# jonassibbesen/rpvg

Measured on AMD Instinct MI355X. Metric: read-pairs quantified/sec, higher is better.
Workload: dtype f64

## Files before the change

### rpvg_amd/csrc/subset_em.hip

```cpp

#include "common.hpp"

#include <cmath>
#include <memory>

using namespace rpvg_hip_detail;

namespace {

constexpr uint32_t kMaxSelected = 1024;

struct MergedList {
    const uint32_t * a;
    const uint32_t * b;
    uint32_t na, nb, i, j;
    __device__ __forceinline__ MergedList(const uint32_t * a_in, uint32_t na_in, const uint32_t * b_in, uint32_t nb_in)
        : a(a_in), b(b_in), na(na_in), nb(nb_in), i(0), j(0) {}
    __device__ __forceinline__ bool done() const { return i >= na && j >= nb; }
    __device__ __forceinline__ uint32_t next() {
        if (j >= nb || (i < na && a[i] <= b[j])) return a[i++];
        return b[j++];
    }
};

// ... 232 lines not shown
        for (uint32_t stride = size >> 1; stride > 0; stride >>= 1) {
            for (uint32_t i = threadIdx.x; i < padded; i += BLOCK) {
                const uint32_t partner = i ^ stride;
                if (partner > i) {
                    const bool ascending = (i & size) == 0;
                    const uint32_t x = order[i], y = order[partner];
                    if (before(y, x) == ascending) {
                        order[i] = y;
                        order[partner] = x;
                    }
                }
            }
            __syncthreads();
        }
    }
    const uint64_t slot0 = args.slot_off[m];
    unsigned long long my_subsets = 0, my_length = 0, my_columns = 0;
    for (uint32_t rank = threadIdx.x; rank < n_ret; rank += BLOCK) {
        const uint32_t s = order[rank];
        uint32_t distinct = 0, previous = 0xffffffffu;
        MergedList walk = columns.list(first[sel[s]], second[sel[s]]);
        while (!walk.done()) {
            const uint32_t path = walk.next();
            distinct += (path != previous) ? 1u : 0u;
            previous = path;
        }
        args.slot_first[slot0 + rank] = first[sel[s]];
        args.slot_second[slot0 + rank] = second[sel[s]];
        args.slot_weight[slot0 + rank] = weight[s];
        args.slot_length[slot0 + rank] = length[s];
        args.slot_columns[slot0 + rank] = distinct;
        my_subsets += 1;
        my_length += length[s];
        my_columns += distinct;
    }
    if (my_subsets) {
        atomicAdd(&red[0], my_subsets);
        atomicAdd(&red[1], my_length);
        atomicAdd(&red[2], my_columns);
    }
    __syncthreads();
    if (threadIdx.x == 0) {
        const uint64_t r0 = args.cluster_row_off[k], r1 = args.cluster_row_off[k + 1];
        const unsigned long long rows = r1 - r0, entries = args.row_ent_off[r1] - args.row_ent_off[r0];
        *out_totals = MatrixTotals{red[0], red[1], red[2], red[0] * rows, red[0] * entries, red[0] * ((rows + args.segment_rows - 1) / args.segment_rows)};
    }
}

__global__ __launch_bounds__(64) void subsetSelectSmallKernel(const SelectArgs args) {
    const uint32_t m = blockIdx.x;
    if (m >= args.num_matrices) return;
    if (args.pair_count[m] > kSmallSelected) {
        if (threadIdx.x == 0) args.big_matrices[atomicAdd(&args.header->big_count, 1u)] = m;
        return;
    }
    selectSubsetsOfMatrix<kSmallSelected, kSmallCachedPaths, 64>(args, m);
}

__global__ __launch_bounds__(256) void subsetSelectWideKernel(const SelectArgs args) {
    const uint32_t count = args.header->big_count;
    for (uint32_t item = blockIdx.x; item < count; item += gridDim.x) {
        selectSubsetsOfMatrix<kMaxSelected, kWideCachedPaths, 256>(args, args.big_matrices[item]);
        __syncthreads();
    }
}

struct OffsetsArgs {
    const uint32_t * pair_count;
    const unsigned long long * log_evals;
    const uint32_t * build_error;
    uint32_t num_matrices;
    const MatrixTotals * totals;
    MatrixTotals * bases;
    SubsetHeader * header;
    unsigned long long cap_subsets, cap_length, cap_columns, cap_rows, cap_entries, cap_items;
    uint64_t * seg_first;
    uint64_t * path_off;
    uint64_t * col_off;
};

__global__ __launch_bounds__(1024) void subsetOffsetsKernel(const OffsetsArgs args) {
    __shared__ MatrixTotals sums[1024];
    const uint32_t M = args.num_matrices;
    const uint32_t per = (M + 1023) / 1024;
    const uint32_t lo = min(M, threadIdx.x * per), hi = min(M, lo + per);
    MatrixTotals mine{0, 0, 0, 0, 0, 0};
    unsigned long long my_pairs = 0;
    for (uint32_t m = lo; m < hi; ++m) {
        my_pairs += args.pair_count[m];
        const MatrixTotals t = args.totals[m];
        mine.subsets += t.subsets;
        mine.list_length += t.list_length;
        mine.columns += t.columns;
        mine.rows += t.rows;
        mine.entries += t.entries;
        mine.segments += t.segments;
    }
    sums[threadIdx.x] = mine;
    if (my_pairs) atomicAdd(&args.header->kept_pairs, my_pairs);
    __syncthreads();
    for (uint32_t step = 1; step < 1024; step <<= 1) {
        MatrixTotals add{0, 0, 0, 0, 0, 0};
        if (threadIdx.x >= step) add = sums[threadIdx.x - step];
        __syncthreads();
        MatrixTotals & s = sums[threadIdx.x];
        s.subsets += add.subsets;
        s.list_length += add.list_length;
        s.columns += add.columns;
        s.rows += add.rows;
        s.entries += add.entries;
        s.segments += add.segments;
        __syncthreads();
    }
    MatrixTotals run = sums[threadIdx.x];
    run.subsets -= mine.subsets;
    run.list_length -= mine.list_length;
    run.columns -= mine.columns;
    run.rows -= mine.rows;
    run.entries -= mine.entries;
    run.segments -= mine.segments;
    for (uint32_t m = lo; m < hi; ++m) {
        args.bases[m] = run;
        const MatrixTotals t = args.totals[m];
        run.subsets += t.subsets;
        run.list_length += t.list_length;
        run.columns += t.columns;
        run.rows += t.rows;
        run.entries += t.entries;
        run.segments += t.segments;
    }
    if (threadIdx.x == 1023) {
        const MatrixTotals all = sums[1023];
        SubsetHeader * h = args.header;
        h->subsets = all.subsets;
        h->list_length = all.list_length;
        h->columns = all.columns;
        h->rows = all.rows;
        h->entries = all.entries;
        h->segments = all.segments;
        const bool fits = h->select_overflow == 0 && all.subsets <= args.cap_subsets && all.list_length <= args.cap_length &&
                          all.columns <= args.cap_columns && all.rows <= args.cap_rows && all.entries <= args.cap_entries &&
                          all.segments <= args.cap_items && all.subsets < 0xffffffffull && all.segments < 0xffffffffull;
        h->overflow = fits ? 0ull : 1ull;
        h->num_problems = fits ? static_cast<uint32_t>(all.subsets) : 0u;
        h->num_items = fits ? static_cast<uint32_t>(all.segments) : 0u;
        h->log_evals = *args.log_evals;
        h->build_bad = args.build_error ? *args.build_error : 0u;
        if (fits) {
            args.path_off[all.subsets] = all.list_length;
            args.col_off[all.subsets] = all.columns;
            args.seg_first[all.subsets] = all.segments;
        }
    }
}

struct ExpandArgs {
    uint32_t num_matrices;
    const SubsetHeader * header;
    const MatrixTotals * totals;
    const MatrixTotals * bases;
    const uint64_t * slot_off;
    const uint32_t * slot_first;
    const uint32_t * slot_second;
    const double * slot_weight;
    const uint32_t * slot_length;
    const uint32_t * slot_columns;
    const uint64_t * group_off;
    const uint64_t * group_path_off;
    const uint32_t * group_path;
    const uint32_t * cluster;
    const uint64_t * cluster_row_off;
    const uint64_t * row_ent_off;
    uint32_t * sub_cluster;
    double * sub_weight;
    uint64_t * path_off;
    uint32_t * path;
    uint64_t * col_off;
    uint32_t * col_path;
    uint64_t * row_base;
    uint64_t * ent_base;
    uint64_t * seg_first;
    uint32_t * item_problem;
    uint32_t segment_rows;
    uint64_t * subset_off;
};

__global__ __launch_bounds__(256) void subsetExpandKernel(const ExpandArgs args) {
    constexpr int BLOCK = 256;
    __shared__ uint32_t scratch[BLOCK / 64];
    const uint32_t m = blockIdx.x;
    if (m >= args.num_matrices) return;
    const MatrixTotals base = args.bases[m];
    if (threadIdx.x == 0) {
        args.subset_off[m] = args.header->overflow ? 0 : base.subsets;
        if (m + 1 == args.num_matrices) args.subset_off[m + 1] = args.header->overflow ? 0 : args.header->subsets;
    }
    if (args.header->overflow) return;
    const uint32_t n = static_cast<uint32_t>(args.totals[m].subsets);
    const uint64_t slot0 = args.slot_off[m];
    const Columns columns{args.group_path_off, args.group_path, args.group_off[m]};
    const uint32_t k = args.cluster[m];
    const uint64_t r0 = args.cluster_row_off[k], r1 = args.cluster_row_off[k + 1];
    const uint64_t rows = r1 - r0, entries = args.row_ent_off[r1] - args.row_ent_off[r0];
    uint64_t length_run = base.list_length, columns_run = base.columns;
    for (uint32_t c = 0; c < n; c += BLOCK) {
        const uint32_t r = c + threadIdx.x;
        const uint32_t len = r < n ? args.slot_length[slot0 + r] : 0u, cols = r < n ? args.slot_columns[slot0 + r] : 0u;
        uint32_t len_total, cols_total;
        const uint32_t len_before = blockExclusiveScan<BLOCK>(len, len_total, scratch);
        const uint32_t cols_before = blockExclusiveScan<BLOCK>(cols, cols_total, scratch);
        if (r < n) {
            const uint64_t s = base.subsets + r;
            const uint64_t p0 = length_run + len_before, c0 = columns_run + cols_before;
            args.sub_cluster[s] = k;
            args.sub_weight[s] = args.slot_weight[slot0 + r];
            args.path_off[s] = p0;
            args.col_off[s] = c0;
            args.row_base[s] = base.rows + static_cast<uint64_t>(r) * rows;
            args.ent_base[s] = base.entries + static_cast<uint64_t>(r) * entries;
            const uint64_t segments = (rows + args.segment_rows - 1) / args.segment_rows, item0 = base.segments + static_cast<uint64_t>(r) * segments;
            args.seg_first[s] = item0;
            for (uint64_t item = item0; item < item0 + segments; ++item) args.item_problem[item] = static_cast<uint32_t>(s);
            MergedList list = columns.list(args.slot_first[slot0 + r], args.slot_second[slot0 + r]);
            uint32_t previous = 0xffffffffu;
            uint64_t pw = p0, cw = c0;
            while (!list.done()) {
                const uint32_t path = list.next();
                args.path[pw++] = path;
                if (path != previous) args.col_path[cw++] = path;
                previous = path;
            }
        }
        length_run += len_total;
        columns_run += cols_total;
    }
}

struct PackArgs {
    const SubsetHeader * header;
    uint32_t num_matrices;
    const uint64_t * subset_off;
    const double * weight;
    const uint64_t * path_off;
    const uint64_t * col_off;
    const double * abundances;
    const double * noise;
    const double * total;
    const uint32_t * path;
    const uint32_t * col_path;
    const uint32_t * iterations;
    const uint32_t * kept_rows;
    const uint32_t * kept_entries;
    const uint32_t * merge_bad;
    unsigned char * packed;
};

__global__ __launch_bounds__(256) void packResultsKernel(const PackArgs args) {
    const SubsetHeader h = *args.header;
    if (h.overflow) return;
    const uint64_t M = args.num_matrices, S = h.subsets, L = h.list_length, C = h.columns;
    const PackedLayout lay = packedLayout(M, S, L, C);
    const size_t stride = static_cast<size_t>(gridDim.x) * blockDim.x, first = static_cast<size_t>(blockIdx.x) * blockDim.x + threadIdx.x;
    auto copy = [&](const size_t offset, const void * from, const size_t words) {
        uint32_t * to = reinterpret_cast<uint32_t *>(args.packed + offset);
        const uint32_t * src = static_cast<const uint32_t *>(from);
        for (size_t i = first; i < words; i += stride) to[i] = src[i];
    };
    copy(lay.subset_off, args.subset_off, (M + 1) * 2);
    copy(lay.weight, args.weight, S * 2);
    copy(lay.path_off, args.path_off, (S + 1) * 2);
    copy(lay.col_off, args.col_off, (S + 1) * 2);
    copy(lay.abundances, args.abundances, C * 2);
    copy(lay.noise, args.noise, S * 2);
    copy(lay.total, args.total, S * 2);
    copy(lay.path, args.path, L);
    copy(lay.col_path, args.col_path, C);
    copy(lay.iterations, args.iterations, S);
    copy(lay.kept_rows, args.kept_rows, S);
    copy(lay.kept_entries, args.kept_entries, S);
    if (args.merge_bad && first == 0) *reinterpret_cast<uint32_t *>(args.packed + lay.merge_flags) = *args.merge_bad;
}

constexpr uint32_t kMergeLdsRecords = 2048;
constexpr unsigned long long kMergeNoRecord = ~0ull;
constexpr uint32_t kMergePathBits = 27, kMergeRankBits = 10;

struct MergeArgs {
    const SubsetHeader * header;
    uint32_t num_matrices;
    const uint64_t * subset_off;
    const double * weight;
    const uint64_t * path_off;
    const uint32_t * path;
    const uint64_t * col_off;
    const uint32_t * col_path;
    const double * abundances;
    const double * noise;
    const double * total;
    const uint32_t * cluster;
    const uint64_t * cluster_path_off;
    const uint32_t * path_group_id;
    unsigned long long * sort_key;
    uint32_t * sort_pos;
    double * rec_a0;
    double * rec_a1;
    uint32_t * merge_bad;
// ... 180 lines not shown
    uint32_t max_paths = 0;
    std::vector<uint64_t> slot_off(M + 1, 0);
    for (uint32_t m = 0; m < M; ++m) {
        const uint64_t G = groups->h_num_cols[m];
        slot_off[m + 1] = slot_off[m] + std::min<uint64_t>(G * (G + 1) / 2, kMaxSelected);
        const uint32_t k = groups->h_cluster[m];
        lane_rows += batch->h_cluster_row_off[k + 1] - batch->h_cluster_row_off[k];
        lane_entries += batch->h_cluster_ent_off[k + 1] - batch->h_cluster_ent_off[k];
        lane_paths += groups->h_num_paths[m];
        max_paths = std::max(max_paths, groups->h_num_paths[m]);
        max_cluster_work = std::max<uint64_t>(max_cluster_work, (batch->h_cluster_row_off[k + 1] - batch->h_cluster_row_off[k]) +
                                                                    (batch->h_cluster_ent_off[k + 1] - batch->h_cluster_ent_off[k]));
    }
    slots = slot_off[M];
    if (M > 0 && 8ull * (5ull * (static_cast<uint64_t>(max_paths) + 1) + 6) > 156 * 1024) {
        setError("rpvg_hip_nested_subset_em: not taken (a cluster with %u paths: EM vectors in global memory)", max_paths);
        return RPVG_HIP_ERR_UNSUPPORTED;
    }

    std::lock_guard<std::mutex> lock(ctx->mutex);
    RPVG_HIP_CHECK(hipSetDevice(ctx->device));
    hipStream_t st = ctx->stream;
    if (M == 0) {
        *result_out = res.release();
        return RPVG_HIP_OK;
    }
    SubsetEmHints & hints = ctx->subset_hints;
    auto planned = [](const double per_unit, const unsigned long long units, const double headroom) {
        return static_cast<unsigned long long>(std::ceil(per_unit * headroom * static_cast<double>(units)));
    };
    unsigned long long cap_subsets = std::min<unsigned long long>(slots, hints.subsets_per_matrix > 0 ? planned(hints.subsets_per_matrix, M, 1.25) + 256 : std::max<unsigned long long>(8ull * M, 16384));
    unsigned long long cap_length = std::max<unsigned long long>(planned(hints.list_per_path, lane_paths, 2.0), std::max<unsigned long long>(8 * lane_paths, 1u << 20));
    unsigned long long cap_rows = hints.rows_per_row > 0 ? planned(hints.rows_per_row, lane_rows, 1.25) + 65536 : 8 * lane_rows;
    unsigned long long cap_entries = hints.entries_per_entry > 0 ? planned(hints.entries_per_entry, lane_entries, 1.25) + 65536 : 8 * lane_entries;
    if (hints.retry) {
        cap_subsets = std::min<unsigned long long>(slots, std::max(cap_subsets, hints.retry_subsets + 64));
        cap_length = std::max(cap_length, hints.retry_list_length + 64);
        cap_rows = std::max(cap_rows, hints.retry_rows + 64);
        cap_entries = std::max(cap_entries, hints.retry_entries + 64);
        hints.retry = false;
    }
    const unsigned long long cap_columns = cap_length;
    const unsigned long long cap_items = cap_rows / emFillSegmentRows() + cap_subsets;

    scope.reset(new HostScope("subset em: search + kernels queued"));
    const size_t header_room = 256;
    int rc = RPVG_HIP_OK;
    if (!second_attempt) {
        search.extra_u64 = slot_off.data();
        search.extra_u64_count = M + 1;
        search.extra_zero_bytes = header_room + emQueuesBytes();
        rc = queuePairSearch(ctx, groups, column_counts, min_rel_likelihood, search);
        if (rc != RPVG_HIP_OK) return rc;
    } else {
        const hipError_t zeroed = zeroAsync(search.d_extra_zero.ptr, search.extra_zero_bytes, st);
        if (zeroed != hipSuccess) {
            setError("rpvg_hip_nested_subset_em: %s", hipGetErrorString(zeroed));
            return RPVG_HIP_ERR_RUNTIME;
        }
    }

    hipError_t e = hipSuccess;
    auto ok = [&](hipError_t r) { if (e == hipSuccess) e = r; return e == hipSuccess; };
    const uint64_t * d_slot_off = search.d_extra_u64.ptr;
    SubsetHeader * header = reinterpret_cast<SubsetHeader *>(search.d_extra_zero.ptr);
    static_assert(sizeof(SubsetHeader) <= 256, "room for the header");
    DeviceBuffer<uint32_t> d_slot_first, d_slot_second, d_slot_length, d_slot_columns;
    DeviceBuffer<double> d_slot_weight;
    DeviceBuffer<unsigned char> d_totals, d_bases, d_packed;
    ok(d_slot_first.alloc(slots));
    ok(d_slot_second.alloc(slots));
    ok(d_slot_length.alloc(slots));
    ok(d_slot_columns.alloc(slots));
    ok(d_slot_weight.alloc(slots));
    ok(d_totals.alloc(sizeof(MatrixTotals) * M));
    ok(d_bases.alloc(sizeof(MatrixTotals) * M));
    DeviceBuffer<uint32_t> d_big_matrices;
    ok(d_big_matrices.alloc(M));
    DeviceBuffer<uint32_t> d_sub_cluster, d_path, d_col_path, d_iters, d_kept_rows, d_kept_entries;
    DeviceBuffer<double> d_sub_weight, d_abund, d_noise, d_total;
    DeviceBuffer<uint64_t> d_path_off, d_col_off, d_row_base, d_ent_base, d_subset_off, d_seg_first;
    DeviceBuffer<uint32_t> d_item_problem;
    ok(d_sub_cluster.alloc(cap_subsets));
    ok(d_sub_weight.alloc(cap_subsets));
    ok(d_path_off.alloc(cap_subsets + 1));
    ok(d_col_off.alloc(cap_subsets + 1));
    ok(d_row_base.alloc(cap_subsets));
    ok(d_ent_base.alloc(cap_subsets));
    ok(d_subset_off.alloc(M + 1));
    ok(d_seg_first.alloc(cap_subsets + 1));
    ok(d_item_problem.alloc(cap_items));
    ok(d_path.alloc(cap_length));
    ok(d_col_path.alloc(cap_columns));
    ok(d_abund.alloc(cap_columns));
    ok(d_noise.alloc(cap_subsets));
    ok(d_total.alloc(cap_subsets));
    ok(d_iters.alloc(cap_subsets));
    ok(d_kept_rows.alloc(cap_subsets));
    ok(d_kept_entries.alloc(cap_subsets));
    const size_t packed_capacity = packedLayout(M, cap_subsets, cap_length, cap_columns).bytes;
    ok(d_packed.alloc(packed_capacity));
    const bool merge_here = batch->path_group_id.ptr != nullptr && max_paths < (1u << kMergePathBits) - 2;
    DeviceBuffer<unsigned long long> d_merge_key;
    DeviceBuffer<uint32_t> d_merge_pos;
    DeviceBuffer<double> d_merge_a0, d_merge_a1;
    if (merge_here) {
        ok(d_merge_key.alloc(2 * cap_length + 2));
        ok(d_merge_pos.alloc(2 * cap_length + 2));
        ok(d_merge_a0.alloc(cap_length));
        ok(d_merge_a1.alloc(cap_length));
    }
    void * pinned_header = nullptr;
    if (e == hipSuccess && pinnedAlloc(&pinned_header, sizeof(SubsetHeader)) != hipSuccess) e = hipErrorOutOfMemory;
    hipEvent_t header_here = nullptr;
    if (e == hipSuccess) ok(hipEventCreateWithFlags(&header_here, hipEventDisableTiming));
    if (e != hipSuccess) {
        setError("rpvg_hip_nested_subset_em: %s", hipGetErrorString(e));
        (void) hipStreamSynchronize(st);
        leavePairSearch(ctx);
        if (pinned_header) pinnedFree(pinned_header);
        if (header_here) (void) hipEventDestroy(header_here);
        return (e == hipErrorOutOfMemory) ? RPVG_HIP_ERR_ALLOC : RPVG_HIP_ERR_RUNTIME;
    }
    MatrixTotals * totals = reinterpret_cast<MatrixTotals *>(d_totals.ptr);
    MatrixTotals * bases = reinterpret_cast<MatrixTotals *>(d_bases.ptr);

    std::unique_ptr<HostScope> part_scope(new HostScope("subset em: select + offsets + expand queued"));
    int span = ctx->spanBegin(FAM_BUILD);
    SelectArgs sa;
    sa.num_matrices = M;
    sa.pair_count = search.d_tail.ptr;
    sa.pair_cap_off = search.d_pair_cap_off.ptr;
    sa.pair_first = search.d_out_first.ptr;
    sa.pair_second = search.d_out_second.ptr;
    sa.pair_value = search.d_out_value.ptr;
    sa.group_off = groups->d_group_off;
    sa.group_path_off = groups->d_group_path_off;
    sa.group_path = groups->d_group_path;
    sa.cluster = groups->d_cluster;
    sa.mat_rows = groups->mat_rows.ptr;
    sa.cluster_row_off = batch->cluster_row_off.ptr;
    sa.row_ent_off = batch->row_ent_off.ptr;
    sa.slot_off = d_slot_off;
    sa.min_hap_prob = min_hap_prob;
    sa.segment_rows = emFillSegmentRows();
    sa.slot_first = d_slot_first.ptr;
    sa.slot_second = d_slot_second.ptr;
    sa.slot_weight = d_slot_weight.ptr;
    sa.slot_length = d_slot_length.ptr;
    sa.slot_columns = d_slot_columns.ptr;
    sa.totals = totals;
    sa.header = header;
    sa.big_matrices = d_big_matrices.ptr;
    subsetSelectSmallKernel<<<dim3(M), dim3(64), 0, st>>>(sa);
    subsetSelectWideKernel<<<dim3(std::min<uint32_t>(M, 128)), dim3(256), 0, st>>>(sa);
    const bool check_build = !groups->build_checked && groups->build_error_flag.ptr;
    OffsetsArgs oa;
    oa.pair_count = search.d_tail.ptr;
    oa.log_evals = reinterpret_cast<const unsigned long long *>(search.d_tail.ptr + search.evals_word);
    oa.build_error = check_build ? groups->build_error_flag.ptr : nullptr;
    oa.num_matrices = M;
    oa.totals = totals;
    oa.bases = bases;
    oa.header = header;
    oa.cap_subsets = cap_subsets;
    oa.cap_length = cap_length;
    oa.cap_columns = cap_columns;
    oa.cap_rows = cap_rows;
    oa.cap_entries = cap_entries;
    oa.cap_items = cap_items;
    oa.seg_first = d_seg_first.ptr;
    oa.path_off = d_path_off.ptr;
    oa.col_off = d_col_off.ptr;
    subsetOffsetsKernel<<<dim3(1), dim3(1024), 0, st>>>(oa);
    SubsetHeader * h_header = static_cast<SubsetHeader *>(pinned_header);
    ok(hipMemcpyAsync(h_header, header, sizeof(SubsetHeader), hipMemcpyDeviceToHost, st));
    ok(hipEventRecord(header_here, st));
    ExpandArgs ea;
    ea.num_matrices = M;
    ea.header = header;
    ea.totals = totals;
    ea.bases = bases;
    ea.slot_off = d_slot_off;
    ea.slot_first = d_slot_first.ptr;
    ea.slot_second = d_slot_second.ptr;
    ea.slot_weight = d_slot_weight.ptr;
    ea.slot_length = d_slot_length.ptr;
    ea.slot_columns = d_slot_columns.ptr;
    ea.group_off = groups->d_group_off;
    ea.group_path_off = groups->d_group_path_off;
    ea.group_path = groups->d_group_path;
    ea.cluster = groups->d_cluster;
    ea.cluster_row_off = batch->cluster_row_off.ptr;
    ea.row_ent_off = batch->row_ent_off.ptr;
    ea.sub_cluster = d_sub_cluster.ptr;
    ea.sub_weight = d_sub_weight.ptr;
    ea.path_off = d_path_off.ptr;
    ea.path = d_path.ptr;
    ea.col_off = d_col_off.ptr;
    ea.col_path = d_col_path.ptr;
    ea.row_base = d_row_base.ptr;
    ea.ent_base = d_ent_base.ptr;
    ea.seg_first = d_seg_first.ptr;
    ea.item_problem = d_item_problem.ptr;
    ea.segment_rows = emFillSegmentRows();
    ea.subset_off = d_subset_off.ptr;
    subsetExpandKernel<<<dim3(M), dim3(256), 0, st>>>(ea);
    ok(hipGetLastError());
    ctx->spanEnd(span);
    ctx->stats.build_launches += 4;
    leavePairSearch(ctx);

    part_scope.reset();
    EmProblemList list;
    list.P_bound = static_cast<uint32_t>(std::min<unsigned long long>(cap_subsets, 0xfffffffeull));
    list.d_num_problems = &header->num_problems;
    list.d_cluster = d_sub_cluster.ptr;
    list.d_col_off = d_col_off.ptr;
    list.d_col_path = d_col_path.ptr;
    list.d_row_base = d_row_base.ptr;
    list.d_ent_base = d_ent_base.ptr;
    list.rows_capacity = cap_rows;
    list.entries_capacity = cap_entries;
    list.d_seg_first = d_seg_first.ptr;
    list.d_item_problem = d_item_problem.ptr;
    list.items_bound = static_cast<uint32_t>(std::min<unsigned long long>(cap_items, 0xfffffffeull));
    list.d_num_items = &header->num_items;
    list.max_cols = max_paths + 1;
    list.max_cluster_paths = max_paths;
    list.max_cluster_work = max_cluster_work;
    list.wide_capacity = 0;
    EmOutputs out{d_abund.ptr, d_noise.ptr, d_iters.ptr, d_kept_rows.ptr, d_kept_entries.ptr, d_total.ptr};
    EmSolveWork work;
    work.zeroed_queues = search.d_extra_zero.ptr + header_room;
    if (e == hipSuccess) {
        rc = queueEmSolve(ctx, batch, list, max_em_its, max_rel_em_conv, out, work, false, collapse_precision);
        if (rc != RPVG_HIP_OK) {
            (void) hipStreamSynchronize(st);
            (void) hipEventDestroy(header_here);
            pinnedFree(pinned_header);
            return rc;
        }
    }
    part_scope.reset(new HostScope("subset em: merge + pack queued"));
    static_assert(sizeof(SubsetHeader) <= 192, "the merge's flag word sits behind the header");
    uint32_t * d_merge_bad = reinterpret_cast<uint32_t *>(search.d_extra_zero.ptr + 192);
    if (merge_here && e == hipSuccess) {
        MergeArgs ma;
        ma.header = header;
        ma.num_matrices = M;
        ma.subset_off = d_subset_off.ptr;
        ma.weight = d_sub_weight.ptr;
        ma.path_off = d_path_off.ptr;
        ma.path = d_path.ptr;
        ma.col_off = d_col_off.ptr;
        ma.col_path = d_col_path.ptr;
        ma.abundances = d_abund.ptr;
        ma.noise = d_noise.ptr;
        ma.total = d_total.ptr;
        ma.cluster = groups->d_cluster;
        ma.cluster_path_off = batch->cluster_path_off.ptr;
        ma.path_group_id = batch->path_group_id.ptr;
        ma.sort_key = d_merge_key.ptr;
        ma.sort_pos = d_merge_pos.ptr;
        ma.rec_a0 = d_merge_a0.ptr;
        ma.rec_a1 = d_merge_a1.ptr;
        ma.merge_bad = d_merge_bad;
        ma.packed = d_packed.ptr;
        const int merge_span = ctx->spanBegin(FAM_BUILD);
        subsetMergeKernel<<<dim3(M), dim3(256), 0, st>>>(ma);
        ctx->spanEnd(merge_span);
        ctx->stats.build_launches += 1;
    }
    PackArgs pa;
    pa.merge_bad = merge_here ? d_merge_bad : nullptr;
    pa.header = header;
    pa.num_matrices = M;
    pa.subset_off = d_subset_off.ptr;
    pa.weight = d_sub_weight.ptr;
    pa.path_off = d_path_off.ptr;
    pa.col_off = d_col_off.ptr;
    pa.abundances = d_abund.ptr;
    pa.noise = d_noise.ptr;
    pa.total = d_total.ptr;
    pa.path = d_path.ptr;
    pa.col_path = d_col_path.ptr;
    pa.iterations = d_iters.ptr;
    pa.kept_rows = d_kept_rows.ptr;
    pa.kept_entries = d_kept_entries.ptr;
    pa.packed = d_packed.ptr;
    packResultsKernel<<<dim3(256), dim3(256), 0, st>>>(pa);
    ok(hipGetLastError());

    part_scope.reset();
    scope.reset(new HostScope("subset em: header"));
    if (e == hipSuccess) ok(waitEvent(header_here));
    (void) hipEventDestroy(header_here);
    if (e != hipSuccess) {
        setError("rpvg_hip_nested_subset_em: %s", hipGetErrorString(e));
        (void) hipStreamSynchronize(st);
        pinnedFree(pinned_header);
        return (e == hipErrorOutOfMemory) ? RPVG_HIP_ERR_ALLOC : RPVG_HIP_ERR_RUNTIME;
    }
    const SubsetHeader got = *h_header;
    pinnedFree(pinned_header);
    {
        auto fold = [](double & kept, const unsigned long long needed, const unsigned long long units) {
            kept = std::max(0.9 * kept, static_cast<double>(needed) / static_cast<double>(std::max<unsigned long long>(units, 1)));
        };
        fold(hints.subsets_per_matrix, got.subsets, M);
        fold(hints.list_per_path, got.list_length, lane_paths);
        fold(hints.rows_per_row, got.rows, lane_rows);
        fold(hints.entries_per_entry, got.entries, lane_entries);
    }
    if (got.build_bad) {
        (void) hipStreamSynchronize(st);
        setError(got.build_bad == 2 ? "rpvg_hip_groups_build: a group lists a path twice" : "rpvg_hip_groups_build: a group refers to a path outside its cluster");
        return RPVG_HIP_ERR_INVALID;
    }
    groups->build_checked = true;
    if (got.overflow) {
        (void) hipStreamSynchronize(st);
        setError("rpvg_hip_nested_subset_em: not taken (%llu subsets, %llu rows, %llu entries, %llu selected-diplotype overflows: over the reserved "
                 "capacity)", got.subsets, got.rows, got.entries, got.select_overflow);
        if (!got.select_overflow) {
            hints.retry = true;
            hints.retry_subsets = got.subsets;
            hints.retry_list_length = std::max(got.list_length, got.columns);
            hints.retry_rows = got.rows;
            hints.retry_entries = got.entries;
            *did_not_fit = true;
        }
        return RPVG_HIP_ERR_UNSUPPORTED;
    }
    scope.reset(new HostScope("subset em: wait for the EM + download"));
    const uint64_t S = got.subsets;
    const PackedLayout lay = packedLayout(M, S, got.list_length, got.columns);
    if (pinnedAlloc(&res->block, std::max<size_t>(lay.bytes, 64)) != hipSuccess) {
        (void) hipStreamSynchronize(st);
        setError("rpvg_hip_nested_subset_em: out of page-locked host memory");
        return RPVG_HIP_ERR_ALLOC;
    }
    unsigned char * host = static_cast<unsigned char *>(res->block);
    ok(hipMemcpyAsync(host, d_packed.ptr, lay.bytes, hipMemcpyDeviceToHost, st));
    ok(waitStream(st));
    if (e != hipSuccess) {
        setError("rpvg_hip_nested_subset_em: %s", hipGetErrorString(e));
        return RPVG_HIP_ERR_RUNTIME;
    }
    accountPairSearch(ctx, groups, search, got.log_evals, got.kept_pairs);

    rpvg_hip_subset_em_view & v = res->view;
    v.num_matrices = M;
    v.subset_off = reinterpret_cast<const uint64_t *>(host + lay.subset_off);
    v.weight = reinterpret_cast<const double *>(host + lay.weight);
    v.path_off = reinterpret_cast<const uint64_t *>(host + lay.path_off);
    v.path = reinterpret_cast<const uint32_t *>(host + lay.path);
    v.col_off = reinterpret_cast<const uint64_t *>(host + lay.col_off);
    v.col_path = reinterpret_cast<const uint32_t *>(host + lay.col_path);
    v.abundances = reinterpret_cast<const double *>(host + lay.abundances);
    v.noise_count = reinterpret_cast<const double *>(host + lay.noise);
    v.total_count = reinterpret_cast<const double *>(host + lay.total);
    v.iterations = reinterpret_cast<const uint32_t *>(host + lay.iterations);
    if (merge_here) {
        if (*reinterpret_cast<const uint32_t *>(host + lay.merge_flags)) {
            setError("rpvg_hip_nested_subset_em: a diplotype's path subset holds more than two paths of one transcript (PathInfo::group_id): "
                     "the reference asserts against it (src/path_abundance_estimator.cpp:722)");
            return RPVG_HIP_ERR_INVALID;
        }
        v.set_count = reinterpret_cast<const uint32_t *>(host + lay.set_count);
        v.cluster_noise_count = reinterpret_cast<const double *>(host + lay.cluster_noise);
        v.set_first = reinterpret_cast<const uint32_t *>(host + lay.set_first);
        v.set_second = reinterpret_cast<const uint32_t *>(host + lay.set_second);
        v.set_posterior = reinterpret_cast<const double *>(host + lay.set_posterior);
        v.set_abundance = reinterpret_cast<const double *>(host + lay.set_abund);
    }
    res->num_subsets = S;
    accountEmSolve(ctx, static_cast<uint32_t>(S), v.col_off, reinterpret_cast<const uint32_t *>(host + lay.kept_rows),
                   reinterpret_cast<const uint32_t *>(host + lay.kept_entries), v.iterations);
    *result_out = res.release();
    return RPVG_HIP_OK;
}

extern "C" int rpvg_hip_nested_subset_em(rpvg_hip_ctx * ctx, const rpvg_hip_batch * batch, const rpvg_hip_groups * groups,
                                         const uint32_t * column_counts, double min_rel_likelihood, double min_hap_prob,
                                         uint32_t max_em_its, double max_rel_em_conv, double collapse_precision,
                                         rpvg_hip_subset_em ** result_out) {
    RPVG_REQUIRE(ctx && batch && groups && result_out, "rpvg_hip_nested_subset_em: NULL argument");
    *result_out = nullptr;
    bool did_not_fit = false;
    PairSearchWork search;
    int rc = nestedSubsetEmAttempt(ctx, batch, groups, column_counts, min_rel_likelihood, min_hap_prob, max_em_its, max_rel_em_conv, collapse_precision,
                                   result_out, &did_not_fit, search, false);
    if (rc == RPVG_HIP_ERR_UNSUPPORTED && did_not_fit) {
        static const bool trace = std::getenv("RPVG_AMD_TRACE") != nullptr;
        if (trace) std::fprintf(stderr, "[rpvg_hip trace]   subset em: second attempt (%s)\n", rpvg_hip_last_error());
        rc = nestedSubsetEmAttempt(ctx, batch, groups, column_counts, min_rel_likelihood, min_hap_prob, max_em_its, max_rel_em_conv, collapse_precision,
                                   result_out, &did_not_fit, search, true);
    }
    return rc;
}

extern "C" int rpvg_hip_subset_em_get(const rpvg_hip_subset_em * result, rpvg_hip_subset_em_view * view_out) {
    RPVG_REQUIRE(result && view_out, "rpvg_hip_subset_em_get: NULL argument");
    *view_out = result->view;
    view_out->num_matrices = result->num_matrices;
    return RPVG_HIP_OK;
}

extern "C" void rpvg_hip_subset_em_free(rpvg_hip_subset_em * result) { delete result; }
```

Measured before the change: 2.417 billion.

## Fuse subset select and offsets kernels into one launch with last-block scan

Replaces the separate small-select, wide-select and offsets kernels with one fused kernel. Wide blocks handle matrices with many pairs, other blocks pack four small matrices per block with one wave each, and the last block to arrive computes the prefix offsets. Column and path lists are staged in LDS when they fit, and the header copy to the host is moved after the expand launch. This removes two launches and the gaps between them, at the cost of a larger LDS footprint per block and an atomic arrival counter.

Measured after the change: 2.316 billion. 4.2% lower.

```diff
diff --git a/rpvg_amd/csrc/subset_em.hip b/rpvg_amd/csrc/subset_em.hip
--- a/rpvg_amd/csrc/subset_em.hip
+++ b/rpvg_amd/csrc/subset_em.hip
@@ -408,6 +408,436 @@
             args.seg_first[all.subsets] = all.segments;
         }
     }
+}
+
+constexpr uint32_t kSelectThreads = 256, kSelectWideBlocks = 128;
+constexpr uint32_t kSmallCachedColumns = 128, kWideCachedColumns = 512;
+
+template <uint32_t CAP, uint32_t CACHE, uint32_t COLS>
+struct SelectLds {
+    union {
+        double value[CAP];
+        unsigned long long key[CAP];
+    };
+    union {
+        unsigned long long hash[CAP];
+        double weight[CAP];
+    };
+    uint32_t first[CAP], second[CAP];
+    uint32_t length[CAP], distinct[CAP];
+    uint32_t leader[CAP];
+    uint32_t order[CAP];
+    uint32_t paths[CACHE];
+    uint32_t col_off[COLS + 1];
+    unsigned long long red[3];
+    double sum_posterior;
+    uint32_t counts[2][4];
+    uint32_t n_retained, max_path;
+};
+
+template <int THREADS>
+__device__ __forceinline__ void selectSync() {
+    if constexpr (THREADS > 64) {
+        __syncthreads();
+    } else {
+        __builtin_amdgcn_fence(__ATOMIC_SEQ_CST, "workgroup");
+        __builtin_amdgcn_wave_barrier();
+    }
+}
+
+template <bool CACHED, typename LDS>
+struct StagedColumns {
+    const LDS & lds;
+    const uint64_t * group_path_off;
+    const uint32_t * group_path;
+    uint64_t first_column;
+    __device__ __forceinline__ MergedList list(const uint32_t first, const uint32_t second) const {
+        if constexpr (CACHED) {
+            const uint32_t a0 = lds.col_off[first], a1 = lds.col_off[first + 1], b0 = lds.col_off[second], b1 = lds.col_off[second + 1];
+            return MergedList(lds.paths + a0, a1 - a0, lds.paths + b0, b1 - b0);
+        } else {
+            const uint64_t a0 = group_path_off[first_column + first], a1 = group_path_off[first_column + first + 1];
+            const uint64_t b0 = group_path_off[first_column + second], b1 = group_path_off[first_column + second + 1];
+            return MergedList(group_path + a0, static_cast<uint32_t>(a1 - a0), group_path + b0, static_cast<uint32_t>(b1 - b0));
+        }
+    }
+};
+
+__device__ __forceinline__ unsigned long long listKey(MergedList list, const bool narrow) {
+    unsigned long long key = 0;
+    const int count = narrow ? 4 : 2, bits = narrow ? 16 : 32;
+    for (int i = 0; i < count; ++i) {
+        key <<= bits;
+        if (!list.done()) key |= static_cast<unsigned long long>(list.next()) + 1ull;
+    }
+    return key;
+}
+
+struct MatrixPlace {
+    uint64_t base, col0, col1, path0, path1;
+    uint32_t cluster;
+    unsigned long long rows, entries;
+};
+
+__device__ __forceinline__ MatrixPlace placeOfMatrix(const SelectArgs & args, const uint32_t m) {
+    MatrixPlace p;
+    p.base = args.pair_cap_off[m];
+    p.col0 = args.group_off[m];
+    p.col1 = args.group_off[m + 1];
+    p.cluster = args.cluster[m];
+    p.path0 = args.group_path_off[p.col0];
+    p.path1 = args.group_path_off[p.col1];
+    const uint64_t r0 = args.cluster_row_off[p.cluster], r1 = args.cluster_row_off[p.cluster + 1];
+    p.rows = r1 - r0;
+    p.entries = args.row_ent_off[r1] - args.row_ent_off[r0];
+    return p;
+}
+
+template <bool CACHED, int THREADS, typename LDS, uint32_t CAP>
+__device__ __forceinline__ void selectStagedSubsets(const SelectArgs & args, const uint32_t m, const uint32_t tid, LDS & lds, const uint32_t n_pairs,
+                                                    const MatrixPlace & place) {
+    const int lane = tid & 63, wave = tid >> 6;
+    const uint64_t base = place.base, col0 = place.col0, path0 = place.path0;
+    const uint32_t n_paths = static_cast<uint32_t>(place.path1 - place.path0);
+    const uint32_t * first_g = args.pair_first + base;
+    const uint32_t * second_g = args.pair_second + base;
+    const double * value_g = args.pair_value + base;
+    const unsigned long long rows = place.rows, entries = place.entries;
+    const double threshold = args.min_hap_prob;
+    MatrixTotals * out_totals = args.totals + m;
+    const StagedColumns<CACHED, LDS> columns{lds, args.group_path_off, args.group_path, col0};
+    double v = tid < n_pairs ? value_g[tid] : 0.0;
+
+    if (tid == 0) {
+        lds.red[0] = lds.red[1] = lds.red[2] = 0;
+        lds.n_retained = 0;
+        lds.max_path = 0;
+    }
+    selectSync<THREADS>();
+    if constexpr (CACHED) {
+        const uint32_t G = static_cast<uint32_t>(place.col1 - col0);
+        for (uint32_t g = tid; g <= G; g += THREADS) lds.col_off[g] = static_cast<uint32_t>(args.group_path_off[col0 + g] - path0);
+        uint32_t largest = 0;
+        for (uint32_t i = tid; i < n_paths; i += THREADS) {
+            const uint32_t path = args.group_path[path0 + i];
+            lds.paths[i] = path;
+            largest = max(largest, path);
+        }
+        if (n_paths > tid) atomicMax(&lds.max_path, largest);
+    }
+    uint32_t n_sel = 0;
+    for (uint32_t c = 0, round = 0; c < n_pairs; c += THREADS, ++round) {
+        const uint32_t i = c + tid;
+        const bool take = i < n_pairs && v >= threshold;
+        const double mine = v;
+        if (i + THREADS < n_pairs) v = value_g[i + THREADS];
+        const unsigned long long ballot = __ballot(take);
+        uint32_t at = n_sel + __popcll(ballot & ((1ull << lane) - 1ull)), total = __popcll(ballot);
+        if constexpr (THREADS > 64) {
+            uint32_t * counts = lds.counts[round & 1];
+            if (lane == 0) counts[wave] = total;
+            __syncthreads();
+            total = 0;
+#pragma unroll
+            for (int w = 0; w < THREADS / 64; ++w) {
+                if (w < wave) at += counts[w];
+                total += counts[w];
+            }
+        }
+        if (take && at < CAP) {
+            lds.value[at] = mine;
+            lds.order[at] = i;
+        }
+        n_sel += total;
+    }
+    if (n_sel > CAP) {
+        if (tid == 0) {
+            atomicAdd(&args.header->select_overflow, 1ull);
+            *out_totals = MatrixTotals{0, 0, 0, 0, 0, 0};
+        }
+        return;
+    }
+    selectSync<THREADS>();
+    for (uint32_t s = tid; s < n_sel; s += THREADS) {
+        const uint32_t i = lds.order[s];
+        lds.first[s] = first_g[i];
+        lds.second[s] = second_g[i];
+    }
+    if (tid == THREADS - 1) {
+        double sum = 0;
+        for (uint32_t s = 0; s < n_sel; ++s) sum += lds.value[s];
+        lds.sum_posterior = sum;
+    }
+    selectSync<THREADS>();
+    for (uint32_t s = tid; s < n_sel; s += THREADS) {
+        MergedList list = columns.list(lds.first[s], lds.second[s]);
+        unsigned long long h = 1469598103934665603ull;
+        uint32_t n = 0, distinct = 0, previous = 0xffffffffu;
+        while (!list.done()) {
+            const uint32_t path = list.next();
+            h = (h ^ path) * 1099511628211ull;
+            ++n;
+            distinct += (path != previous) ? 1u : 0u;
+            previous = path;
+        }
+        lds.hash[s] = h;
+        lds.length[s] = n;
+        lds.distinct[s] = distinct;
+    }
+    selectSync<THREADS>();
+    for (uint32_t s = tid; s < n_sel; s += THREADS) {
+        const unsigned long long h = lds.hash[s];
+        uint32_t lead = s;
+        for (uint32_t t = 0; t < s; ++t) {
+            if (lds.hash[t] == h && lds.length[t] == lds.length[s] &&
+                compareLists(columns.list(lds.first[t], lds.second[t]), columns.list(lds.first[s], lds.second[s])) == 0) {
+                lead = t;
+                break;
+            }
+        }
+        lds.leader[s] = lead;
+    }
+    selectSync<THREADS>();
+    const double sum_posterior = lds.sum_posterior;
+    double my_weight[(CAP + THREADS - 1) / THREADS];
+#pragma unroll
+    for (uint32_t j = 0; j < (CAP + THREADS - 1) / THREADS; ++j) {
+        const uint32_t s = tid + j * THREADS;
+        double w = 0;
+        if (s < n_sel && lds.leader[s] == s) {
+            for (uint32_t t = s; t < n_sel; ++t) {
+                if (lds.leader[t] == s) w += lds.value[t];
+            }
+            w /= sum_posterior;
+        }
+        my_weight[j] = w;
+    }
+    selectSync<THREADS>();
+    const bool narrow = CACHED && lds.max_path < 0xffffu;
+#pragma unroll
+    for (uint32_t j = 0; j < (CAP + THREADS - 1) / THREADS; ++j) {
+        const uint32_t s = tid + j * THREADS;
+        if (s < n_sel) {
+            const bool leads = lds.leader[s] == s;
+            lds.weight[s] = my_weight[j];
+            if (leads && my_weight[j] >= threshold) {
+                lds.key[s] = listKey(columns.list(lds.first[s], lds.second[s]), narrow);
+                lds.order[atomicAdd(&lds.n_retained, 1u)] = s;
+            }
+        }
+    }
+    selectSync<THREADS>();
+    const uint32_t n_ret = lds.n_retained;
+    auto before = [&](const uint32_t x, const uint32_t y) {
+        if (x == 0xffffffffu) return false;
+        if (y == 0xffffffffu) return true;
+        const unsigned long long kx = lds.key[x], ky = lds.key[y];
+        if (kx != ky) return kx < ky;
+        return compareLists(columns.list(lds.first[x], lds.second[x]), columns.list(lds.first[y], lds.second[y])) < 0;
+    };
+    const uint32_t * ranked = lds.order;
+    if (n_ret <= 64) {
+        if (tid < n_ret) {
+            const uint32_t s = lds.order[tid];
+            uint32_t rank = 0;
+            for (uint32_t q = 0; q < n_ret; ++q) rank += (q != tid && before(lds.order[q], s)) ? 1u : 0u;
+            lds.leader[rank] = s;
+        }
+        ranked = lds.leader;
+        selectSync<THREADS>();
+    } else {
+        uint32_t padded = 1;
+        while (padded < n_ret) padded <<= 1;
+        for (uint32_t i = n_ret + tid; i < padded; i += THREADS) lds.order[i] = 0xffffffffu;
+        selectSync<THREADS>();
+        for (uint32_t size = 2; size <= padded; size <<= 1) {
+            for (uint32_t stride = size >> 1; stride > 0; stride >>= 1) {
+                for (uint32_t i = tid; i < padded; i += THREADS) {
+                    const uint32_t partner = i ^ stride;
+                    if (partner > i) {
+                        const bool ascending = (i & size) == 0;
+                        const uint32_t x = lds.order[i], y = lds.order[partner];
+                        if (before(y, x) == ascending) {
+                            lds.order[i] = y;
+                            lds.order[partner] = x;
+                        }
+                    }
+                }
+                selectSync<THREADS>();
+            }
+        }
+    }
+    const uint64_t slot0 = args.slot_off[m];
+    unsigned long long my_subsets = 0, my_length = 0, my_columns = 0;
+    for (uint32_t rank = tid; rank < n_ret; rank += THREADS) {
+        const uint32_t s = ranked[rank];
+        args.slot_first[slot0 + rank] = lds.first[s];
+        args.slot_second[slot0 + rank] = lds.second[s];
+        args.slot_weight[slot0 + rank] = lds.weight[s];
+        args.slot_length[slot0 + rank] = lds.length[s];
+        args.slot_columns[slot0 + rank] = lds.distinct[s];
+        my_subsets += 1;
+        my_length += lds.length[s];
+        my_columns += lds.distinct[s];
+    }
+    if (my_subsets) {
+        atomicAdd(&lds.red[0], my_subsets);
+        atomicAdd(&lds.red[1], my_length);
+        atomicAdd(&lds.red[2], my_columns);
+    }
+    selectSync<THREADS>();
+    if (tid == 0) {
+        const unsigned long long n = lds.red[0];
+        *out_totals = MatrixTotals{n, lds.red[1], lds.red[2], n * rows, n * entries, n * ((rows + args.segment_rows - 1) / args.segment_rows)};
+    }
+}
+
+template <int THREADS, typename LDS, uint32_t CAP, uint32_t CACHE, uint32_t COLS>
+__device__ __forceinline__ void selectSubsetsStaged(const SelectArgs & args, const uint32_t m, const uint32_t tid, LDS & lds, const uint32_t n_pairs,
+                                                    const MatrixPlace & place) {
+    if (place.path1 - place.path0 <= CACHE && place.col1 - place.col0 <= COLS) {
+        selectStagedSubsets<true, THREADS, LDS, CAP>(args, m, tid, lds, n_pairs, place);
+    } else {
+        selectStagedSubsets<false, THREADS, LDS, CAP>(args, m, tid, lds, n_pairs, place);
+    }
+}
+
+template <int THREADS>
+__device__ __forceinline__ void offsetsOfTheMatrices(const OffsetsArgs & args, unsigned long long (*wave_sums)[6]) {
+    const int lane = threadIdx.x & 63, wave = threadIdx.x >> 6;
+    const uint32_t M = args.num_matrices;
+    const uint32_t per = (M + THREADS - 1) / THREADS;
+    const uint32_t lo = min(M, threadIdx.x * per), hi = min(M, lo + per);
+    unsigned long long mine[6] = {0, 0, 0, 0, 0, 0}, my_pairs = 0;
+    uint32_t my_big = 0;
+    for (uint32_t m = lo; m < hi; ++m) {
+        const uint32_t pairs = args.pair_count[m];
+        my_pairs += pairs;
+        my_big += pairs > kSmallSelected ? 1u : 0u;
+        const MatrixTotals t = args.totals[m];
+        mine[0] += t.subsets;
+        mine[1] += t.list_length;
+        mine[2] += t.columns;
+        mine[3] += t.rows;
+        mine[4] += t.entries;
+        mine[5] += t.segments;
+    }
+    if (my_pairs) atomicAdd(&args.header->kept_pairs, my_pairs);
+    if (my_big) atomicAdd(&args.header->big_count, my_big);
+    unsigned long long run[6];
+#pragma unroll
+    for (int f = 0; f < 6; ++f) {
+        unsigned long long incl = mine[f];
+#pragma unroll
+        for (int d = 1; d < 64; d <<= 1) {
+            const unsigned long long up = __shfl_up(incl, d, 64);
+            if (lane >= d) incl += up;
+        }
+        if (lane == 63) wave_sums[wave][f] = incl;
+        run[f] = incl - mine[f];
+    }
+    __syncthreads();
+    unsigned long long all[6];
+#pragma unroll
+    for (int f = 0; f < 6; ++f) {
+        all[f] = 0;
+#pragma unroll
+        for (int w = 0; w < THREADS / 64; ++w) {
+            if (w < wave) run[f] += wave_sums[w][f];
+            all[f] += wave_sums[w][f];
+        }
+    }
+    for (uint32_t m = lo; m < hi; ++m) {
+        args.bases[m] = MatrixTotals{run[0], run[1], run[2], run[3], run[4], run[5]};
+        const MatrixTotals t = args.totals[m];
+        run[0] += t.subsets;
+        run[1] += t.list_length;
+        run[2] += t.columns;
+        run[3] += t.rows;
+        run[4] += t.entries;
+        run[5] += t.segments;
+    }
+    if (threadIdx.x == THREADS - 1) {
+        SubsetHeader * h = args.header;
+        h->subsets = all[0];
+        h->list_length = all[1];
+        h->columns = all[2];
+        h->rows = all[3];
+        h->entries = all[4];
+        h->segments = all[5];
+        const bool fits = atomicAdd(&h->select_overflow, 0ull) == 0 && all[0] <= args.cap_subsets && all[1] <= args.cap_length &&
+                          all[2] <= args.cap_columns && all[3] <= args.cap_rows && all[4] <= args.cap_entries &&
+                          all[5] <= args.cap_items && all[0] < 0xffffffffull && all[5] < 0xffffffffull;
+        h->overflow = fits ? 0ull : 1ull;
+        h->num_problems = fits ? static_cast<uint32_t>(all[0]) : 0u;
+        h->num_items = fits ? static_cast<uint32_t>(all[5]) : 0u;
+        h->log_evals = *args.log_evals;
+        h->build_bad = args.build_error ? *args.build_error : 0u;
+        if (fits) {
+            args.path_off[all[0]] = all[1];
+            args.col_off[all[0]] = all[2];
+            args.seg_first[all[0]] = all[5];
+        }
+    }
+}
+
+struct FusedSelectArgs {
+    SelectArgs select;
+    OffsetsArgs offsets;
+    uint32_t wide_blocks;
+    uint32_t * arrivals;
+};
+
+using WideSelectLds = SelectLds<kMaxSelected, kWideCachedPaths, kWideCachedColumns>;
+using SmallSelectLds = SelectLds<kSmallSelected, kSmallCachedPaths, kSmallCachedColumns>;
+
+__global__ __launch_bounds__(kSelectThreads) void subsetSelectKernel(const FusedSelectArgs args) {
+    __shared__ union {
+        WideSelectLds wide;
+        SmallSelectLds small[kSelectThreads / 64];
+        unsigned long long wave_sums[kSelectThreads / 64][6];
+    } lds;
+    __shared__ unsigned long long wide_here[kSelectThreads / 64];
+    __shared__ uint32_t arrived_before;
+    const SelectArgs & sa = args.select;
+    const uint32_t M = sa.num_matrices, W = args.wide_blocks;
+    const int lane = threadIdx.x & 63, wave = threadIdx.x >> 6;
+    if (blockIdx.x < W) {
+        for (uint32_t first = blockIdx.x; first < M; first += W * kSelectThreads) {
+            const uint64_t mine = first + static_cast<uint64_t>(threadIdx.x) * W;
+            const unsigned long long ballot = __ballot(mine < M && sa.pair_count[mine < M ? mine : 0] > kSmallSelected);
+            if (lane == 0) wide_here[wave] = ballot;
+            __syncthreads();
+            for (uint32_t w = 0; w < kSelectThreads / 64; ++w) {
+                unsigned long long left = wide_here[w];
+                while (left) {
+                    const uint32_t bit = __ffsll(left) - 1;
+                    left &= left - 1;
+                    const uint32_t m = first + (w * 64 + bit) * W;
+                    selectSubsetsStaged<kSelectThreads, WideSelectLds, kMaxSelected, kWideCachedPaths, kWideCachedColumns>(sa, m, threadIdx.x, lds.wide, sa.pair_count[m],
+                                                                                                                           placeOfMatrix(sa, m));
+                    __syncthreads();
+                }
+            }
+            __syncthreads();
+        }
+    } else {
+        const uint64_t m = __builtin_amdgcn_readfirstlane(static_cast<uint32_t>(blockIdx.x - W) * (kSelectThreads / 64) + wave);
+        if (m < M) {
+            const uint32_t n_pairs = sa.pair_count[m];
+            const MatrixPlace place = placeOfMatrix(sa, static_cast<uint32_t>(m));
+            if (n_pairs <= kSmallSelected) {
+                selectSubsetsStaged<64, SmallSelectLds, kSmallSelected, kSmallCachedPaths, kSmallCachedColumns>(sa, static_cast<uint32_t>(m), lane, lds.small[wave], n_pairs, place);
+            }
+        }
+    }
+    __threadfence();
+    __syncthreads();
+    if (threadIdx.x == 0) arrived_before = atomicAdd(args.arrivals, 1u);
+    __syncthreads();
+    if (arrived_before + 1 != gridDim.x) return;
+    __threadfence();
+    offsetsOfTheMatrices<kSelectThreads>(args.offsets, lds.wave_sums);
 }
 
 struct ExpandArgs {
@@ -894,8 +1324,11 @@
     sa.totals = totals;
     sa.header = header;
     sa.big_matrices = d_big_matrices.ptr;
-    subsetSelectSmallKernel<<<dim3(M), dim3(64), 0, st>>>(sa);
-    subsetSelectWideKernel<<<dim3(std::min<uint32_t>(M, 128)), dim3(256), 0, st>>>(sa);
+    static const bool separate_select = RPVG_EXPERIMENT_ENV("RPVG_HIP_SELECT_SEPARATE") != nullptr;
+    if (separate_select) {
+        subsetSelectSmallKernel<<<dim3(M), dim3(64), 0, st>>>(sa);
+        subsetSelectWideKernel<<<dim3(std::min<uint32_t>(M, 128)), dim3(256), 0, st>>>(sa);
+    }
     const bool check_build = !groups->build_checked && groups->build_error_flag.ptr;
     OffsetsArgs oa;
     oa.pair_count = search.d_tail.ptr;
@@ -914,10 +1347,24 @@
     oa.seg_first = d_seg_first.ptr;
     oa.path_off = d_path_off.ptr;
     oa.col_off = d_col_off.ptr;
-    subsetOffsetsKernel<<<dim3(1), dim3(1024), 0, st>>>(oa);
+    if (separate_select) {
+        subsetOffsetsKernel<<<dim3(1), dim3(1024), 0, st>>>(oa);
+    } else {
+        static_assert(sizeof(SubsetHeader) <= 192 && header_room >= 212, "the arrival counter sits behind the header and the merge's flag word");
+        FusedSelectArgs fa;
+        fa.select = sa;
+        fa.offsets = oa;
+        static const uint32_t wide_blocks = RPVG_EXPERIMENT_ENV("RPVG_HIP_SELECT_WIDE_BLOCKS") ? std::max(1, std::atoi(RPVG_EXPERIMENT_ENV("RPVG_HIP_SELECT_WIDE_BLOCKS"))) : kSelectWideBlocks;
+        fa.wide_blocks = std::min<uint32_t>(M, wide_blocks);
+        fa.arrivals = reinterpret_cast<uint32_t *>(search.d_extra_zero.ptr + 208);
+        subsetSelectKernel<<<dim3(fa.wide_blocks + (M + kSelectThreads / 64 - 1) / (kSelectThreads / 64)), dim3(kSelectThreads), 0, st>>>(fa);
+    }
     SubsetHeader * h_header = static_cast<SubsetHeader *>(pinned_header);
-    ok(hipMemcpyAsync(h_header, header, sizeof(SubsetHeader), hipMemcpyDeviceToHost, st));
-    ok(hipEventRecord(header_here, st));
+    static const bool copy_first = separate_select || RPVG_EXPERIMENT_ENV("RPVG_HIP_SELECT_COPY_FIRST") != nullptr;
+    if (copy_first) {
+        ok(hipMemcpyAsync(h_header, header, sizeof(SubsetHeader), hipMemcpyDeviceToHost, st));
+        ok(hipEventRecord(header_here, st));
+    }
     ExpandArgs ea;
     ea.num_matrices = M;
     ea.header = header;
@@ -950,8 +1397,12 @@
     subsetExpandKernel<<<dim3(M), dim3(256), 0, st>>>(ea);
     ok(hipGetLastError());
     ctx->spanEnd(span);
-    ctx->stats.build_launches += 4;
+    ctx->stats.build_launches += separate_select ? 4 : 2;
     leavePairSearch(ctx);
+    if (!copy_first) {
+        ok(hipMemcpyAsync(h_header, header, sizeof(SubsetHeader), hipMemcpyDeviceToHost, st));
+        ok(hipEventRecord(header_here, st));
+    }
 
     part_scope.reset();
     EmProblemList list;
@@ -1045,6 +1496,7 @@
         return (e == hipErrorOutOfMemory) ? RPVG_HIP_ERR_ALLOC : RPVG_HIP_ERR_RUNTIME;
     }
     const SubsetHeader got = *h_header;
+    if (RPVG_EXPERIMENT_ENV("RPVG_HIP_SELECT_DEBUG")) fprintf(stderr, "select: %u matrices, %u wide, %llu kept pairs, %llu subsets\n", M, got.big_count, got.kept_pairs, got.subsets);
     pinnedFree(pinned_header);
     {
         auto fold = [](double & kept, const unsigned long long needed, const unsigned long long units) {
```
